# SonSang/dmesh2_renderer

Hardware: AMD Instinct MI355X
Metric: Mpixels/s fwd+bwd @1080p/1M tris (higher is better)
Workload: dtype f32

## Files before the change

dmesh2_renderer_amd/csrc/dm2_forward_queue.hip:

```cpp
#include <hip/hip_runtime.h>

#include "dm2_clip_area.h"
#include "dm2_device_math.h"
#include "dm2_pairs.h"
#include "dm2_stage.h"
#include "dm2_stamps.h"
#include "dm2_state.h"

namespace dm2 {

#ifndef DM2_FQ_CHUNK
#define DM2_FQ_CHUNK 52
#endif
#ifndef DM2_FQ_BLOCKS
#define DM2_FQ_BLOCKS 4
#endif
#ifndef DM2_FQ_PAIRCAP
#define DM2_FQ_PAIRCAP 768
#endif
#ifndef DM2_FQ_SURVCAP
#define DM2_FQ_SURVCAP 512
#endif
constexpr int FQ_CHUNK = DM2_FQ_CHUNK;
constexpr int FQ_PAIRCAP = DM2_FQ_PAIRCAP;
constexpr int FQ_SURVCAP = DM2_FQ_SURVCAP;
#ifndef DM2_FQ_TAILMIN
#define DM2_FQ_TAILMIN 0
#endif
constexpr int FQ_TAILMIN = DM2_FQ_TAILMIN;
constexpr int FQ_QCAP = ((FQ_PAIRCAP + 3) / 4 + 63) & ~63;
static_assert(FQ_CHUNK <= 64, "one mask bit per staged face; the id window is one wave wide");
constexpr int FQ_REC_CHUNKS = (int)(sizeof(FaceRec) / 16);
static_assert(FQ_PAIRCAP >= TILE_PIX && FQ_SURVCAP >= TILE_PIX, "a single face may own 256 pairs");
static_assert(FQ_PAIRCAP < 65536, "16-bit slots");
static_assert(FQ_SURVCAP == 2 * TILE_PIX && FQ_SURVCAP % 64 == 0 && FQ_QCAP <= 256, "one blend bit per survivor record; 8 bits of record index per queue entry");

constexpr uint32_t QF_REC = 1u;
constexpr uint32_t QF_BLEND = 2u;

struct __attribute__((aligned(8))) FqPair { float alpha, c0, c1, c2, depth; uint32_t flags; };

template <bool CLASSES, bool WEIGHTS>
__global__ void __launch_bounds__(TILE_PIX, DM2_FQ_BLOCKS)
k_render_forward_queue(dm2_render_desc d, const uint2* __restrict__ ranges, const uint32_t* __restrict__ face_list,
                       ImageState is, float* __restrict__ out_color, float* __restrict__ out_depth,
                       int32_t* __restrict__ out_tri_cnt, uint64_t* __restrict__ hit_masks,
                       uint32_t* __restrict__ hit_valid, float* __restrict__ pool, uint32_t pool_cap,
                       uint32_t* __restrict__ hit_base, float* __restrict__ face_weights STAMP_PARAM) {
    __shared__ FaceRec recs[FQ_CHUNK];
    __shared__ uint32_t s_ids[64];
    __shared__ FqPair s_pair[FQ_SURVCAP];
    __shared__ float s_ray[TILE_PIX * 6];
    __shared__ int s_off[FQ_CHUNK + 1];
    __shared__ uint32_t s_rect[FQ_CHUNK];
    __shared__ int s_kb[FQ_CHUNK];
    __shared__ int s_wtot[4];
    __shared__ int s_inv[17];
    __shared__ uint16_t s_slot[FQ_PAIRCAP];
    __shared__ uint32_t s_queue[4 * FQ_QCAP];
    __shared__ unsigned long long s_mask[TILE_PIX];
    __shared__ __attribute__((aligned(16))) unsigned long long s_bmask[FQ_CHUNK * 4];
    __shared__ int s_wtotc[4];
    __shared__ __attribute__((aligned(16))) uint32_t s_rcnt[8];
    __shared__ unsigned long long s_blend[FQ_SURVCAP / 64];
    __shared__ int s_bpre[4][FQ_SURVCAP / 64];
    __shared__ uint32_t s_cbase;
    __shared__ uint32_t s_maxlc;
    __shared__ float s_w[WEIGHTS ? FQ_CHUNK : 1];

    const uint32_t gx = (d.W + TILE - 1) / TILE, gy = (d.H + TILE - 1) / TILE;
    uint32_t tile;
    if (!tile_of_block(gx * gy * (uint32_t)d.B, is.tile_order, tile)) return;
    const int b = (int)(tile / (gx * gy));
    const uint32_t tyx = tile - (uint32_t)b * gx * gy;
    const int tile_y = (int)(tyx / gx), tile_x = (int)(tyx - (uint32_t)tile_y * gx);
    const int tid = threadIdx.x, lane = tid & 63, wid = tid >> 6;
    STAMP_DECL
    fill_inv_table(s_inv);
    s_mask[tid] = 0;
    if constexpr (WEIGHTS) { if (tid < FQ_CHUNK) s_w[tid] = 0.f; }
    if (hit_valid && blockIdx.x == 0 && tid == 0) hit_valid[0] = pool ? 3u : 2u;
    const int lx = tid & 15, ly = tid >> 4;
    const int X0 = tile_x * TILE, Y0 = tile_y * TILE;
    const uint32_t px = X0 + lx, py = Y0 + ly;
    const bool inside = (px < (uint32_t)d.W) && (py < (uint32_t)d.H);
    const int64_t pix = ((int64_t)b * d.H + py) * d.W + px;
    const uint32_t pmx = (uint32_t)d.patch_min[2 * b], pmy = (uint32_t)d.patch_min[2 * b + 1];
    const int X0a = X0 + (int)pmx, Y0a = Y0 + (int)pmy;
    const int xlim = min(TILE - 1, d.W - 1 - X0), ylim = min(TILE - 1, d.H - 1 - Y0);

    if (inside) {
        f3 ro, rd;
        pixel_ray(d, b, pix, px + pmx, py + pmy, d.full_W, d.full_H, ro, rd);
        s_ray[tid * 6] = ro.x; s_ray[tid * 6 + 1] = ro.y; s_ray[tid * 6 + 2] = ro.z;
        s_ray[tid * 6 + 3] = rd.x; s_ray[tid * 6 + 4] = rd.y; s_ray[tid * 6 + 5] = rd.z;
    }
    const uint2 range = ranges[tile];
    const int total = (int)(range.y - range.x);
    const uint4* const grecs = is.face_recs + (int64_t)b * d.F * FACE_REC_U4;
    const int rl = lane / FQ_REC_CHUNKS, rp = lane - rl * FQ_REC_CHUNKS;
    auto request_ids = [&](int nb) {
        if (wid == 2 && nb + lane < total) glds4(face_list + range.x + nb + lane, &s_ids[0]);
    };
    auto request_recs = [&](int nb) {
        const int nc2 = min(FQ_CHUNK, total - nb);
        for (int r0 = 4 * wid; r0 < nc2; r0 += 16) {
            const int r = r0 + rl;
            if (rl < 4 && r < nc2) glds16(grecs + (int64_t)s_ids[r] * FACE_REC_U4 + rp, &recs[r0]);
        }
    };
    if (total > 0) {
        request_ids(0);
        lds_prefetch_wait();
        __syncthreads();
        request_recs(0);
    }
    const float temp = d.aa_temperature;
    const bool use_aa = temp > 0.0f;
    const float pix_area = 1.0f;
    const int K = d.K;

    bool done = !inside;
    float pT = 1.0f, T = 1.0f;
    uint32_t last_contributor = 0;
    float C0 = 0.f, C1 = 0.f, C2 = 0.f, D = 0.f;
    int rec_cnt = 0;
    auto flush_weights = [&](int wb, int wn) {
        if (tid < wn) {
            const float w = s_w[tid];
            if (w != 0.0f) { atomicAdd(face_weights + (int64_t)b * d.F + face_list[range.x + wb + tid], w); s_w[tid] = 0.f; }
        }
    };

    STAMP(0)
    int n = 0;
    for (int base = 0; base < total; base += n) {
        lds_prefetch_wait();
        if constexpr (WEIGHTS) {
            const int ndone = __syncthreads_count(done);
            flush_weights(base - n, n);
            if (ndone == TILE_PIX) break;
        } else if (__syncthreads_count(done) == TILE_PIX) {
            break;
        }
        STAMP(1)
        n = min(FQ_CHUNK, total - base);
        const bool last_chunk = base + n >= total;
        int cnt = 0;
        if (tid < n) {
            uint32_t rect;
            cnt = face_pixel_rect(recs[tid].aa.bb, use_aa, X0a, Y0a, xlim, ylim, rect);
            s_rect[tid] = rect;
        }
        if (tid < FQ_CHUNK * 4) s_bmask[tid] = 0;
        if (tid < FQ_SURVCAP / 64) s_blend[tid] = 0;
        STAMP(2)
        if (wid == 0) {
            const int inc = wave_inclusive_scan(cnt);
            if (tid < n) {
                const int ex = inc - cnt;
                s_off[tid] = ex;
                const uint32_t r = s_rect[tid];
                s_kb[tid] = ex - (int)((r >> 4) & 15u) * ((int)((r >> 8) & 15u) + 1) - (int)(r & 15u);
            }
            if (lane == 63) s_off[n] = inc;
        }
        __syncthreads();
        int tot = s_off[n];
        if (tot > FQ_PAIRCAP) {
            n = find_face(s_off, n, FQ_PAIRCAP);
            tot = s_off[n];
        }
        STAMP(3)

        const int Q = (((tot + 3) >> 2) + 63) & ~63;
        int wcount = 0, wfull = 0;
        for (int r = 0; r < Q; r += 64) {
            const int k = wid * Q + r + lane;
            bool surv = false, full = false;
            uint32_t entry = 0;
            if (k < tot) {
                const int j = find_face(s_off, n, k);
                int qx, qy;
                pair_xy(s_rect[j], k - s_off[j], s_inv, qx, qy);
                uint32_t cmask = 0xF;
                surv = true;
                if (use_aa) {
                    const float pxmin = (float)(uint32_t)(X0a + qx), pymin = (float)(uint32_t)(Y0a + qy);
                    surv = classify_pixel(recs[j].aa, pxmin, pxmin + 1, pymin, pymin + 1, cmask);
                }
                full = surv && (cmask == 0xFu);
                entry = (uint32_t)(qy * TILE + qx) | ((uint32_t)j << 8) | (cmask << 14);
            }
            const unsigned long long bal = __ballot(surv);
            const int before = wcount + (int)__builtin_amdgcn_mbcnt_hi((uint32_t)(bal >> 32), __builtin_amdgcn_mbcnt_lo((uint32_t)bal, 0u));
            if (k < tot) s_slot[k] = (uint16_t)before;
            if (CLASSES) {
                const unsigned long long balf = __ballot(full), balc = bal & ~balf;
                const int rf = wfull + (int)__builtin_amdgcn_mbcnt_hi((uint32_t)(balf >> 32), __builtin_amdgcn_mbcnt_lo((uint32_t)balf, 0u));
                const int rc = (wcount - wfull) + (int)__builtin_amdgcn_mbcnt_hi((uint32_t)(balc >> 32), __builtin_amdgcn_mbcnt_lo((uint32_t)balc, 0u));
                if (surv) s_queue[wid * FQ_QCAP + (full ? FQ_QCAP - 1 - rf : rc)] = entry | ((uint32_t)before << 18);
                wfull += __popcll(balf);
            } else if (surv) s_queue[wid * FQ_QCAP + before] = entry;
            wcount += __popcll(bal);
        }
        if (lane == 0) { s_wtot[wid] = wcount; if (CLASSES) s_wtotc[wid] = wcount - wfull; }
        __syncthreads();
        STAMP(4)
        const int wb1 = s_wtot[0], wb2 = wb1 + s_wtot[1], wb3 = wb2 + s_wtot[2];
        int S = wb3 + s_wtot[3];
        const int ST0 = S;
        int wc1 = 0, wc2 = 0, wc3 = 0, SC = 0;
        if (CLASSES) { wc1 = s_wtotc[0]; wc2 = wc1 + s_wtotc[1]; wc3 = wc2 + s_wtotc[2]; SC = wc3 + s_wtotc[3]; }
        const int wf1 = wb1 - wc1, wf2 = wb2 - wc2, wf3 = wb3 - wc3;
        auto surv_before = [&](int k) -> int {
            if (k >= tot) return S;
            const int w = (k >= Q) + (k >= 2 * Q) + (k >= 3 * Q);
            return (w == 0 ? 0 : (w == 1 ? wb1 : (w == 2 ? wb2 : wb3))) + (int)s_slot[k];
        };
        int target = S;
        if (S > FQ_SURVCAP) target = FQ_SURVCAP;
        else if (FQ_TAILMIN > 0 && !last_chunk && S > TILE_PIX && (S & (TILE_PIX - 1)) != 0 && (S & (TILE_PIX - 1)) < FQ_TAILMIN) target = S & ~(TILE_PIX - 1);
        if (target < S) {
            int lo = 1, hi = n;
            while (hi - lo > 1) {
                const int mid = (lo + hi) >> 1;
                if (surv_before(s_off[mid]) <= target) lo = mid; else hi = mid;
            }
            const int S2 = surv_before(s_off[lo]);
            n = lo; tot = s_off[lo]; S = S2;
        }

        if (base + n < total) request_ids(base + n);
        uint32_t cbase = 0;
        if (pool && tid == 0) cbase = atomicAdd(hit_valid + 1, (uint32_t)S);
        constexpr int FQ_ROUNDS = CLASSES ? (FQ_PAIRCAP + TILE_PIX - 1) / TILE_PIX : FQ_SURVCAP / TILE_PIX;
        const int ST = CLASSES ? ST0 : S;
        float pool_ratio[FQ_ROUNDS];
        int pool_s[FQ_ROUNDS];
#pragma unroll
        for (int rnd = 0; rnd < FQ_ROUNDS; rnd++) { pool_ratio[rnd] = 0.f; pool_s[rnd] = -1; }
        if (!CLASSES && pool && lane == 0) s_rcnt[4 + wid] = 0;
#pragma unroll
        for (int rnd = 0; rnd < FQ_ROUNDS; rnd++) {
            if (rnd * TILE_PIX >= ST) break;
            const int t = tid + rnd * TILE_PIX;
            uint32_t entry = 0u;
            int s = t;
            if (CLASSES) {
                const bool isc = t < SC;
                const int tc = isc ? t : t - SC;
                const int b1 = isc ? wc1 : wf1, b2 = isc ? wc2 : wf2, b3 = isc ? wc3 : wf3;
                const int w = (tc >= b1) + (tc >= b2) + (tc >= b3);
                const int within = tc - (w == 0 ? 0 : (w == 1 ? b1 : (w == 2 ? b2 : b3)));
                if (t < ST) entry = s_queue[w * FQ_QCAP + (isc ? within : FQ_QCAP - 1 - within)];
                s = (w == 0 ? 0 : (w == 1 ? wb1 : (w == 2 ? wb2 : wb3))) + (int)((entry >> 18) & 255u);
            } else if (t < ST) {
                const int w = (s >= wb1) + (s >= wb2) + (s >= wb3);
                entry = s_queue[w * FQ_QCAP + (s - (w == 0 ? 0 : (w == 1 ? wb1 : (w == 2 ? wb2 : wb3))))];
            }
            bool blend_s = false;
            if (t < ST && s < S) {
            const int q = (int)(entry & 255u), j = (int)((entry >> 8) & 63u);
            const uint32_t cmask = (entry >> 14) & 15u;
            const FaceRec& fc = recs[j];
            const float pxmin = (float)(uint32_t)(X0a + (q & 15)), pxmax = pxmin + 1;
            const float pymin = (float)(uint32_t)(Y0a + (q >> 4)), pymax = pymin + 1;
            float oarea = 0.f;
            bool live = true;
            if (use_aa) {
                const int err = clip_area_classified(fc.aa, pxmin, pxmax, pymin, pymax, cmask, pix_area, oarea);
                live = !((err != 0) | (oarea == 0.0f));
            }
            float ratio = oarea / pix_area;
            const f3 ro = {s_ray[q * 6], s_ray[q * 6 + 1], s_ray[q * 6 + 2]};
            const f3 rd = {s_ray[q * 6 + 3], s_ray[q * 6 + 4], s_ray[q * 6 + 5]};
            const f3 p0 = {fc.v[0], fc.v[1], fc.v[2]}, p1 = {fc.v[3], fc.v[4], fc.v[5]}, p2 = {fc.v[6], fc.v[7], fc.v[8]};
            f3 tuv;
            const bool hit = ray_tri_intersection_pred(ro, rd, p0, p1, p2, tuv);
            float iuc, ivc; int code;
            clamp_bary_uv(tuv.y, tuv.z, iuc, ivc, code);
            const float i0 = 1 - iuc - ivc, i1 = iuc, i2 = ivc;
            ratio = mix_coverage(code, ratio, temp);
            blend_s = live & hit & (ratio != 0.0f);
            const float c0 = i0 * fc.col[0] + i1 * fc.col[3] + i2 * fc.col[6];
            const float c1 = i0 * fc.col[1] + i1 * fc.col[4] + i2 * fc.col[7];
            const float c2 = i0 * fc.col[2] + i1 * fc.col[5] + i2 * fc.col[8];
            FqPair out;
            out.c0 = blend_s ? c0 * fc.intense : 0.f; out.c1 = blend_s ? c1 * fc.intense : 0.f; out.c2 = blend_s ? c2 * fc.intense : 0.f;
            out.depth = blend_s ? i0 * fc.dep[0] + i1 * fc.dep[1] + i2 * fc.dep[2] : 0.f;
            out.alpha = blend_s ? fc.opacity * ratio : 0.f;
            out.flags = ((use_aa & live) ? QF_REC : 0u) | (blend_s ? QF_BLEND : 0u);
            if (blend_s) {
                pool_ratio[rnd] = ratio;
                if (CLASSES) { pool_s[rnd] = s; if (pool) atomicOr(&s_blend[s >> 6], 1ull << (s & 63)); }
            }
            if (out.flags) {
                s_pair[s] = out;
                atomicOr(&s_mask[q], 1ull << j);
                if (hit_masks && blend_s) atomicOr(&s_bmask[j * 4 + (q >> 6)], 1ull << (q & 63));
            }
            }
            if (!CLASSES && pool) {
                const unsigned long long bal = __ballot(blend_s);
                pool_s[rnd] = blend_s ? (int)__builtin_amdgcn_mbcnt_hi((uint32_t)(bal >> 32), __builtin_amdgcn_mbcnt_lo((uint32_t)bal, 0u)) : -1;
                if (lane == 0) s_rcnt[rnd * 4 + wid] = __popcll(bal);
            }
        }
        STAMP(5)
        if (pool && tid == 0) s_cbase = cbase;
        lds_prefetch_wait();
        __syncthreads();
        if (base + n < total) request_recs(base + n);
        if (hit_masks && tid < n * 4) hit_masks[((int64_t)range.x + base + (tid >> 2)) * 4 + (tid & 3)] = s_bmask[tid];
        if (pool) {
            const uint32_t cb = s_cbase;
            if (wid == 0) {
                int cj = 0;
                if (lane < n) {
                    const ulonglong2 m01 = reinterpret_cast<const ulonglong2*>(s_bmask)[2 * lane], m23 = reinterpret_cast<const ulonglong2*>(s_bmask)[2 * lane + 1];
                    cj = __popcll(m01.x) + __popcll(m01.y) + __popcll(m23.x) + __popcll(m23.y);
                }
                const int ex = wave_inclusive_scan(cj) - cj;
                if (lane < n) hit_base[(int64_t)range.x + base + lane] = cb + (uint32_t)ex;
            }
            if (!CLASSES) {
                const uint4 c03 = reinterpret_cast<const uint4*>(s_rcnt)[0], c47 = reinterpret_cast<const uint4*>(s_rcnt)[1];
                const uint32_t r0 = (wid > 0 ? c03.x : 0u) + (wid > 1 ? c03.y : 0u) + (wid > 2 ? c03.z : 0u);
                const uint32_t r1 = c03.x + c03.y + c03.z + c03.w + (wid > 0 ? c47.x : 0u) + (wid > 1 ? c47.y : 0u) + (wid > 2 ? c47.z : 0u);
                if (pool_s[0] >= 0) { const uint32_t slot = cb + r0 + (uint32_t)pool_s[0]; if (slot < pool_cap) pool[slot] = pool_ratio[0]; }
                if (FQ_ROUNDS > 1 && pool_s[FQ_ROUNDS > 1 ? 1 : 0] >= 0) { const uint32_t slot = cb + r1 + (uint32_t)pool_s[1]; if (slot < pool_cap) pool[slot] = pool_ratio[1]; }
            } else {
            {
                const int c = lane < FQ_SURVCAP / 64 ? __popcll(s_blend[lane < FQ_SURVCAP / 64 ? lane : 0]) : 0;
                const int ex = wave_inclusive_scan(c) - c;
                if (lane < FQ_SURVCAP / 64) s_bpre[wid][lane] = ex;
                __builtin_amdgcn_fence(__ATOMIC_SEQ_CST, "wavefront");
            }
#pragma unroll
            for (int rnd = 0; rnd < FQ_ROUNDS; rnd++) {
                const int s = pool_s[rnd];
                if (s >= 0) {
                    const uint32_t slot = cb + (uint32_t)(s_bpre[wid][s >> 6] + __popcll(s_blend[s >> 6] & ((1ull << (s & 63)) - 1ull)));
                    if (slot < pool_cap) pool[slot] = pool_ratio[rnd];
                }
            }
            }
        }

        {
            unsigned long long m = s_mask[tid];
            s_mask[tid] = 0;
            while (m && !done) {
                const int j = __ffsll((long long)m) - 1;
                m &= m - 1;
                const int k = s_kb[j] + ly * ((int)((s_rect[j] >> 8) & 15u) + 1) + lx;
                const FqPair pr = s_pair[surv_before(k)];
                if ((pr.flags & QF_REC) && rec_cnt < K) rec_cnt++;
                if (!(pr.flags & QF_BLEND)) continue;
                const float alpha = pr.alpha;
                const float test_T = T * (1 - alpha);
                if constexpr (WEIGHTS) atomicAdd(&s_w[j], alpha * T);
                C0 += pr.c0 * alpha * T; C1 += pr.c1 * alpha * T; C2 += pr.c2 * alpha * T;
                D += pr.depth * alpha * T;
                pT = T; T = test_T;
                last_contributor = (uint32_t)(base + j + 1);
                if (T < T_EPS) done = true;
            }
        }
        STAMP(6)
    }

    if (tid == 0) s_maxlc = 0;
    __syncthreads();
    if constexpr (WEIGHTS) flush_weights(total - n, n);
    { const uint32_t m = wave_inclusive_max(last_contributor); if (lane == 63 && m) atomicMax(&s_maxlc, m); }
    __syncthreads();
    if (tid == 0) is.tile_max_lc[tile] = s_maxlc;
    if (inside) {
        is.final_prev_T[pix] = pT;
        is.final_T[pix] = T;
        is.n_contrib[pix] = last_contributor;
        out_color[3 * pix] = C0 + T * d.background[0];
        out_color[3 * pix + 1] = C1 + T * d.background[1];
        out_color[3 * pix + 2] = C2 + T * d.background[2];
        out_depth[pix] = D + T * 1.0f;
        if (out_tri_cnt) out_tri_cnt[pix] = rec_cnt;
    }
    STAMP(7)
    STAMP_FLUSH
}

void launch_render_forward_queue(const dm2_render_desc& d, const uint2* ranges, const uint32_t* face_list, ImageState is,
                                 float* out_color, float* out_depth, int32_t* out_tri_cnt, uint64_t* hit_masks,
                                 uint32_t* hit_valid, float* pool, int64_t pool_cap, uint32_t* hit_base, bool classes,
                                 float* face_weights, hipStream_t st) {
    const uint32_t Tn = (uint32_t)(((d.W + TILE - 1) / TILE) * ((d.H + TILE - 1) / TILE) * d.B);
    StageTimer tm(ST_FWD, st);
#define DM2_FQ_LAUNCH(C, W)                                                                                                 \
    hipLaunchKernelGGL((k_render_forward_queue<C, W>), dim3(tile_grid_blocks(Tn)), dim3(TILE_PIX), 0, st, d, ranges, face_list, \
                       is, out_color, out_depth, out_tri_cnt, hit_masks, hit_valid, pool, (uint32_t)pool_cap, hit_base,      \
                       face_weights STAMP_ARG(0))
    if (classes) {
        if (face_weights) DM2_FQ_LAUNCH(true, true); else DM2_FQ_LAUNCH(true, false);
    } else {
        if (face_weights) DM2_FQ_LAUNCH(false, true); else DM2_FQ_LAUNCH(false, false);
    }
#undef DM2_FQ_LAUNCH
}

}
```

dmesh2_renderer_amd/csrc/dm2_pairs.h:

```cpp
#pragma once
#include "dm2_device_math.h"

namespace dm2 {

__host__ __device__ __forceinline__ uint32_t tile_grid_blocks(uint32_t Tn) { return 8u * ((Tn + 7u) / 8u); }
__device__ __forceinline__ bool tile_of_block(uint32_t Tn, const uint32_t* __restrict__ order, uint32_t& tile) {
    const uint32_t per = (Tn + 7u) / 8u;
    tile = order[(blockIdx.x & 7u) * per + (blockIdx.x >> 3)];
    return tile < Tn;
}

__device__ __forceinline__ uint32_t pack_rect(int x0, int y0, int w, int h) {
    return (uint32_t)x0 | ((uint32_t)y0 << 4) | ((uint32_t)(w - 1) << 8) | ((uint32_t)(h - 1) << 12);
}

__device__ __forceinline__ int face_pixel_rect(const float bb[4], bool use_bbox, int X0a, int Y0a, int xlim, int ylim,
                                               uint32_t& rect) {
    int x0 = 0, x1 = xlim, y0 = 0, y1 = ylim;
    if (use_bbox) {
        if (!(bb[0] == bb[0]) || !(bb[1] == bb[1]) || !(bb[2] == bb[2]) || !(bb[3] == bb[3])) { rect = 0; return 0; }
        const float lo_x = fminf(fmaxf(ceilf(bb[0]) - 1.0f - (float)X0a, -1.0f), 17.0f);
        const float hi_x = fminf(fmaxf(floorf(bb[1]) - (float)X0a, -1.0f), 17.0f);
        const float lo_y = fminf(fmaxf(ceilf(bb[2]) - 1.0f - (float)Y0a, -1.0f), 17.0f);
        const float hi_y = fminf(fmaxf(floorf(bb[3]) - (float)Y0a, -1.0f), 17.0f);
        x0 = max(x0, (int)lo_x); x1 = min(x1, (int)hi_x);
        y0 = max(y0, (int)lo_y); y1 = min(y1, (int)hi_y);
    }
    if (x1 < x0 || y1 < y0) { rect = 0; return 0; }
    rect = pack_rect(x0, y0, x1 - x0 + 1, y1 - y0 + 1);
    return (x1 - x0 + 1) * (y1 - y0 + 1);
}

__device__ __forceinline__ int wave_inclusive_scan(int v) {
    v += __builtin_amdgcn_update_dpp(0, v, 0x111, 0xF, 0xF, true);
    v += __builtin_amdgcn_update_dpp(0, v, 0x112, 0xF, 0xF, true);
    v += __builtin_amdgcn_update_dpp(0, v, 0x114, 0xF, 0xF, true);
    v += __builtin_amdgcn_update_dpp(0, v, 0x118, 0xF, 0xF, true);
    v += __builtin_amdgcn_update_dpp(0, v, 0x142, 0xA, 0xF, false);
    v += __builtin_amdgcn_update_dpp(0, v, 0x143, 0xC, 0xF, false);
    return v;
}
__device__ __forceinline__ uint32_t wave_inclusive_max(uint32_t u) {
    int v = (int)u;
    v = max(v, __builtin_amdgcn_update_dpp(0, v, 0x111, 0xF, 0xF, true));
    v = max(v, __builtin_amdgcn_update_dpp(0, v, 0x112, 0xF, 0xF, true));
    v = max(v, __builtin_amdgcn_update_dpp(0, v, 0x114, 0xF, 0xF, true));
    v = max(v, __builtin_amdgcn_update_dpp(0, v, 0x118, 0xF, 0xF, true));
    v = max(v, __builtin_amdgcn_update_dpp(0, v, 0x142, 0xA, 0xF, false));
    v = max(v, __builtin_amdgcn_update_dpp(0, v, 0x143, 0xC, 0xF, false));
    return (uint32_t)v;
}

__device__ __forceinline__ int block_exclusive_scan(int v, int* s_wave, int& total) {
    const int lane = threadIdx.x & 63, wid = threadIdx.x >> 6;
    int inc = v;
#pragma unroll
    for (int d = 1; d < 64; d <<= 1) {
        const int t = __shfl_up(inc, d);
        if (lane >= d) inc += t;
    }
    if (lane == 63) s_wave[wid] = inc;
    __syncthreads();
    const int w0 = s_wave[0], w1 = s_wave[1], w2 = s_wave[2], w3 = s_wave[3];
    const int base = (wid > 0 ? w0 : 0) + (wid > 1 ? w1 : 0) + (wid > 2 ? w2 : 0);
    total = w0 + w1 + w2 + w3;
    return base + inc - v;
}

__device__ __forceinline__ int find_face_in(const int* off, int lo, int hi, int k) {
    while (hi - lo > 1) {
        const int mid = (lo + hi) >> 1;
        if (off[mid] <= k) lo = mid; else hi = mid;
    }
    return lo;
}
__device__ __forceinline__ int find_face(const int* off, int n, int k) { return find_face_in(off, 0, n, k); }

__device__ __forceinline__ void fill_inv_table(int* inv_w) {
    if (threadIdx.x >= 1 && threadIdx.x <= 16) inv_w[threadIdx.x] = (65536 + (int)threadIdx.x - 1) / (int)threadIdx.x;
}
__device__ __forceinline__ void pair_xy(uint32_t rect, int local, const int* inv_w, int& lx, int& ly) {
    const int w = (int)((rect >> 8) & 15u) + 1;
    const int inv = inv_w[w];
    const int dy = (local * inv) >> 16;
    lx = (int)(rect & 15u) + (local - dy * w);
    ly = (int)((rect >> 4) & 15u) + dy;
}

__device__ __forceinline__ int pixel_pair(uint32_t rect, int off, int lx, int ly) {
    const int dx = lx - (int)(rect & 15u), dy = ly - (int)((rect >> 4) & 15u);
    const int w = (int)((rect >> 8) & 15u) + 1, h = (int)((rect >> 12) & 15u) + 1;
    if ((unsigned)dx >= (unsigned)w || (unsigned)dy >= (unsigned)h) return -1;
    return off + dy * w + dx;
}

}
```

Baseline: 1083.

## Replace per-pair binary search with per-wave face start bitmap decode tables

```diff
diff --git a/dmesh2_renderer_amd/csrc/dm2_forward_queue.hip b/dmesh2_renderer_amd/csrc/dm2_forward_queue.hip
--- a/dmesh2_renderer_amd/csrc/dm2_forward_queue.hip
+++ b/dmesh2_renderer_amd/csrc/dm2_forward_queue.hip
@@ -33,6 +33,7 @@
 constexpr int FQ_REC_CHUNKS = (int)(sizeof(FaceRec) / 16);
 static_assert(FQ_PAIRCAP >= TILE_PIX && FQ_SURVCAP >= TILE_PIX, "a single face may own 256 pairs");
 static_assert(FQ_PAIRCAP < 65536, "16-bit slots");
+static_assert(FQ_PAIRCAP <= 1024 && FQ_QCAP / 64 <= 4 && 4 * (64 + 4) * 8 <= FQ_SURVCAP * 24, "decode tables: 10 bits of first pair per entry, four start words per wave, four tables inside the pair records");
 static_assert(FQ_SURVCAP == 2 * TILE_PIX && FQ_SURVCAP % 64 == 0 && FQ_QCAP <= 256, "one blend bit per survivor record; 8 bits of record index per queue entry");
 
 constexpr uint32_t QF_REC = 1u;
@@ -171,18 +172,49 @@
             n = find_face(s_off, n, FQ_PAIRCAP);
             tot = s_off[n];
         }
+        const int f_off = lane < n ? s_off[lane] : 0;
+        const int f_pairs = lane < n ? s_off[lane + 1] - f_off : 0;
+        const uint32_t f_rect = lane < n ? s_rect[lane] : 0u;
+        const int Q = (((tot + 3) >> 2) + 63) & ~63;
+        uint2* const dtab = reinterpret_cast<uint2*>(s_pair) + __builtin_amdgcn_readfirstlane(wid) * (64 + 4);
+        unsigned long long* const dbm = reinterpret_cast<unsigned long long*>(dtab + 64);
+        const bool stage = lane < n && f_pairs > 0;
+        const int rel = f_off - wid * Q;
+        if (lane < 4) dbm[lane] = 0ull;
+        {
+            const unsigned long long ne = __ballot(stage);
+            const int rank = (int)__builtin_amdgcn_mbcnt_hi((uint32_t)(ne >> 32), __builtin_amdgcn_mbcnt_lo((uint32_t)ne, 0u));
+            if (stage) {
+                dtab[rank] = make_uint2((uint32_t)lane | ((uint32_t)f_off << 6) | (f_rect << 16), (uint32_t)s_inv[((f_rect >> 8) & 15u) + 1]);
+                if ((uint32_t)rel < (uint32_t)Q) atomicOr(&dbm[rel >> 6], 1ull << (rel & 63));
+            }
+        }
+        int pre = __popcll(__ballot(stage && rel < 0)) - 1;
+        __builtin_amdgcn_fence(__ATOMIC_SEQ_CST, "wavefront");
         STAMP(3)
 
-        const int Q = (((tot + 3) >> 2) + 63) & ~63;
+        uint2 dec[FQ_QCAP / 64];
+#pragma unroll
+        for (int i = 0; i < FQ_QCAP / 64; i++) {
+            const unsigned long long word = dbm[i];
+            const int rank = pre + (int)__builtin_amdgcn_mbcnt_hi((uint32_t)(word >> 32), __builtin_amdgcn_mbcnt_lo((uint32_t)word, 0u)) + (int)((word >> lane) & 1ull);
+            pre += __popcll(word);
+            dec[i] = dtab[max(rank, 0)];
+        }
         int wcount = 0, wfull = 0;
-        for (int r = 0; r < Q; r += 64) {
+#pragma unroll
+        for (int i = 0; i < FQ_QCAP / 64; i++) {
+            const int r = i * 64;
+            if (r >= Q) break;
             const int k = wid * Q + r + lane;
             bool surv = false, full = false;
             uint32_t entry = 0;
             if (k < tot) {
-                const int j = find_face(s_off, n, k);
-                int qx, qy;
-                pair_xy(s_rect[j], k - s_off[j], s_inv, qx, qy);
+                const uint2 e = dec[i];
+                const int j = (int)(e.x & 63u), local = k - (int)((e.x >> 6) & 1023u);
+                const int w = (int)((e.x >> 24) & 15u) + 1;
+                const int dy = (local * (int)e.y) >> 16;
+                const int qx = (int)((e.x >> 16) & 15u) + (local - dy * w), qy = (int)((e.x >> 20) & 15u) + dy;
                 uint32_t cmask = 0xF;
                 surv = true;
                 if (use_aa) {
diff --git a/dmesh2_renderer_amd/csrc/dm2_pairs.h b/dmesh2_renderer_amd/csrc/dm2_pairs.h
--- a/dmesh2_renderer_amd/csrc/dm2_pairs.h
+++ b/dmesh2_renderer_amd/csrc/dm2_pairs.h
@@ -79,13 +79,6 @@
 __device__ __forceinline__ void fill_inv_table(int* inv_w) {
     if (threadIdx.x >= 1 && threadIdx.x <= 16) inv_w[threadIdx.x] = (65536 + (int)threadIdx.x - 1) / (int)threadIdx.x;
 }
-__device__ __forceinline__ void pair_xy(uint32_t rect, int local, const int* inv_w, int& lx, int& ly) {
-    const int w = (int)((rect >> 8) & 15u) + 1;
-    const int inv = inv_w[w];
-    const int dy = (local * inv) >> 16;
-    lx = (int)(rect & 15u) + (local - dy * w);
-    ly = (int)((rect >> 4) & 15u) + dy;
-}
 
 __device__ __forceinline__ int pixel_pair(uint32_t rect, int off, int lx, int ly) {
     const int dx = lx - (int)(rect & 15u), dy = ly - (int)((rect >> 4) & 15u);
```

After: 1104 (median of 6 runs). +1.9%, better.
